# pikapuma/QuBLAS

Hardware: AMD Instinct MI355X
Metric: int-MAC/s (2*M*N*K/s) for Qgemul 4096^3 int<8,8>; % of MI355X int8 peak (higher is better)
Workload: dtype i8 limbs -> i32/i64; 1 GPU; 4096^3 Qgemul int<8,8> signed, linear class (MulArgs int17/frac16, AddArgs Qu<29,16>, C Qu<23,8>), 3x3 int8-limb MFMA; M_per_gpu=4096, N=4096, K=4096, class=linear

## Files before the change

### include/qgemul.h

```cpp
#ifndef QGEMUL_H_
#define QGEMUL_H_

#include <stddef.h>
#include <stdint.h>

#ifdef __cplusplus
extern "C" {
#endif

#define QGEMUL_ABI_VERSION 1u
#define QG_MAX_LEVELS 40

enum {
    QG_RND_POS_INF = 0,
    QG_RND_NEG_INF = 1,
    QG_RND_ZERO = 2,
    QG_RND_INF = 3,
    QG_RND_CONV = 4,
    QG_TRN_TCPL = 5,
    QG_TRN_SMGN = 6
};

enum {
    QG_SAT_TCPL = 0,
// ... 51 lines not shown
} qgemul_desc;

typedef struct qgemul_opts {
    int64_t lda, ldb, ldc;
    int32_t device;
    uint32_t flags;
} qgemul_opts;

enum {
    QG_OPT_FORCE_TREE = 1u,
    QG_OPT_CHECK_RANGE = 2u,
    QG_OPT_GENERIC_TREE = 4u,
    QG_OPT_RUNTIME_MODES = 8u,
    QG_OPT_FUSED_EPILOGUE = 16u,
    QG_OPT_UNFUSED_EPILOGUE = 32u,
    QG_OPT_GENERIC_LAYOUT = 64u,
    QG_OPT_SCHOOLBOOK_LIMBS = 2048u,
    QG_OPT_ARITHMETIC_CONV = 256u,
    QG_OPT_ALL_DEVICES = 512u,
    QG_OPT_BALANCED_LIMBS = 1024u,
    QG_OPT_LOCKSTEP_TILES = 128u,
    QG_OPT_APPROX_GENERAL = 4096u,
    QG_OPT_BATCHED_STACKED = 8192u,
    QG_OPT_BATCHED_TREE = 16384u
};

enum {
    QG_OK = 0,
    QG_EINVAL = -1,
    QG_EUNSUPPORTED = -2,
    QG_EHIP = -3,
    QG_ERCCL = -4,
    QG_ERANGE = -5,
    QG_ENOGPU = -6
};

enum {
    QG_CLASS_LINEAR = 1,
    QG_CLASS_TREE = 2
};

typedef struct qgemul_info {
    int32_t cls;
    int32_t supported;
    int32_t max_bits;
    int32_t in_bits[2];
    int32_t limbs[2];
// ... 255 lines not shown
```

### qublas_amd/build.py

```python
from __future__ import annotations

import os
import subprocess
import sys

HERE = os.path.dirname(os.path.abspath(__file__))
CSRC = os.path.join(HERE, "csrc")
SOURCES = ["qg_api.hip", "qg_run.hip", "qg_pack.hip", "qg_combine_bd.hip", "qg_eltwise.hip", "qg_approx.hip", "qg_eltwise_cplx.hip", "qg_tree.hip", "qg_tree_fast.hip", "qg_tree_fast_bd.hip", "qg_tree64.hip", "qg_tree_cplx.hip", "qg_tree_cplx_bd.hip", "qg_tree_rc.hip", "qg_gemv.hip", "qg_mfma.hip", "qg_mfma_ep_bd.hip", "qg_mfma_grp.hip", "qg_mfma_ep_grp.hip", "qg_mfma_pp.hip", "qg_mfma_ppl.hip", "qg_mfma_k6.hip", "qg_mfma_ring.hip", "qg_comm.hip", "qg_plan.cpp", "qg_geom.cpp"]
HEADERS = ["qg_ops.h", "qg_forms.h", "qg_plan.h", "qg_kernels.h", "qg_geom.h", "qg_tile_walk.h", "qg_grp.h", "qg_mfma_tile.h", "qg_member_forms.h", "qg_mfma_body.h", "qg_ring.h", "qg_step_all.h", "qg_tree_counter.h", "qg_tree_io.h", "qg_tree_bd.h", "qg_eltwise.h", "qg_eltwise_args.h", "qg_approx.h", "qg_approx_dev.h", "qg_cmul.h", "qg_fix.h", "qg_api_int.h", "qg_run_key.h", os.path.join("..", "..", "include", "qgemul.h")]
INCLUDED_UNITS = {"qg_tree_fast_bd.hip": ["qg_tree_fast.hip"], "qg_tree_cplx_bd.hip": ["qg_tree_cplx.hip"]}
FLAGS = ["--offload-arch=gfx950", "-O3", "-std=c++17", "-fPIC", "-Wall", "-Wno-unused-function", "-Wno-unused-value", "-Wno-unused-result", "-x", "hip"]
LIB = os.path.join(HERE, "libqugemm.so")
LIB_DIAG = os.path.join(HERE, "libqugemm_diag.so")


def _stale(obj: str, deps) -> bool:
    if not os.path.exists(obj):
        return True
    t = os.path.getmtime(obj)
    return any(os.path.getmtime(d) > t for d in deps if os.path.exists(d))


def build(force: bool = False, verbose: bool = False, diag: bool = False) -> str:
    hipcc = os.environ.get("HIPCC", "/opt/rocm/bin/hipcc")
    hdrs = [os.path.join(CSRC, h) for h in HEADERS]
    objdir = os.path.join(HERE, "build", "diag") if diag else os.path.join(HERE, "build")
    LIB = LIB_DIAG if diag else globals()["LIB"]
    os.makedirs(objdir, exist_ok=True)
    objs = []
    procs = []
    for s in SOURCES:
        src = os.path.join(CSRC, s)
# ... 21 lines not shown
```

### qublas_amd/capi.py

```python
from __future__ import annotations

import ctypes as C
import os
from typing import Optional

import numpy as np

from .desc import (QG_MAX_EW, Qcomplex, Qu, host_layout, qfmt, qgemul_approx, qgemul_approx_form, qgemul_approx_seg, qgemul_batched_ep, batched_ep, qgemul_grouped_ep, grouped_ep, qgemul_grouped_member, qgemul_cmul, qgemul_cmul_form, qgemul_desc, qgemul_ep_args, qgemul_epilogue,
                   qgemul_epilogue_cplx, qgemul_ew_stage, qgemul_info, qgemul_opts)

_HERE = os.path.dirname(os.path.abspath(__file__))
LIB_PATH = os.path.join(_HERE, "libqugemm_diag.so" if os.environ.get("QUBLAS_AMD_DIAG") == "1" else "libqugemm.so")

QG_OK, QG_EINVAL, QG_EUNSUPPORTED, QG_EHIP, QG_ERCCL, QG_ERANGE, QG_ENOGPU = 0, -1, -2, -3, -4, -5, -6
OPT_FORCE_TREE, OPT_CHECK_RANGE, OPT_GENERIC_TREE, OPT_RUNTIME_MODES, OPT_FUSED_EPILOGUE, OPT_UNFUSED_EPILOGUE = 1, 2, 4, 8, 16, 32
OPT_GENERIC_LAYOUT, OPT_LOCKSTEP_TILES, OPT_ARITHMETIC_CONV, OPT_ALL_DEVICES = 64, 128, 256, 512
OPT_SCHOOLBOOK_LIMBS = 2048
OPT_APPROX_GENERAL = 4096
OPT_BATCHED_TREE = 16384
OPT_BATCHED_STACKED = 8192
OPT_BALANCED_LIMBS = 1024
OPERAND_A, OPERAND_B, OPERAND_C = 0, 1, 2
BITS_ASCII, BITS_PACKED = 0, 1
KERNEL_NAMES = {0: "none", 1: "mfma_i8", 2: "mfma_i8_limb", 3: "tree_i32", 4: "tree_i64", 5: "tree_cplx", 6: "tree_cplx_i32", 7: "mfma_cplx", 8: "gemv_i32", 9: "gemv_i64", 10: "tree_i128", 11: "tree_rc_i32", 12: "mfma_rc"}
CMUL_NAMES = {0: "none", 1: "basic", 2: "tf", 3: "real_a", 4: "real_b"}

EXPORTS = [
    "qgemul_classify", "qgemul_strerror", "qgemul_abi_version", "qgemul_last_hip_error", "qgemul_run",
    "qgemul_ctx_create", "qgemul_ctx_destroy", "qgemul_ctx_sync", "qgemul_ctx_stream",
    "qgemul_plan_create", "qgemul_plan_destroy", "qgemul_plan_info",
    "qgemul_dev_alloc", "qgemul_dev_free", "qgemul_memcpy_h2d", "qgemul_memcpy_d2h",
    "qgemul_pack", "qgemul_pack_f64", "qgemul_unpack_c", "qgemul_execute", "qgemul_fill_packed", "qgemul_time_execute",
    "qgemul_classify_ep", "qgemul_plan_create_ep", "qgemul_packed_e_bytes", "qgemul_pack_e", "qgemul_execute_ep",
    "qgemul_time_execute_ep", "qgemul_run_ep", "qgemul_plan_fuses_epilogue", "qgemul_plan_packed_layout", "qgemul_classify_epc", "qgemul_plan_create_epc", "qgemul_run_epc",
    "qgemul_bitstream_bytes", "qgemul_export_bitstream", "qgemul_run_release", "qgemul_run_sharded", "qgemul_execute_host_c", "qgemul_plan_stores_host_c",
    "qgemul_comm_unique_id", "qgemul_comm_create", "qgemul_comm_destroy", "qgemul_comm_info", "qgemul_gather_packed_c", "qgemul_comm_fence",
    "qgemul_comm_sync", "qgemul_comm_barrier", "qgemul_comm_max_f64", "qgemul_last_rccl_error", "qgemul_ctx_device",
    "qgemul_classify_epx", "qgemul_plan_create_epx", "qgemul_run_epx", "qgemul_plan_approx_uniform", "qgemul_sizeof", "qgemul_approx_plan_form", "qgemul_apply_epilogue", "qgemul_time_apply_epilogue", "qgemul_packed_c_bytes", "qgemul_pack_c",
    "qgemul_classify_epcx", "qgemul_plan_create_epcx", "qgemul_run_epcx", "qgemul_cmul_plan_form",
    "qgemul_classify_batched", "qgemul_classify_batched_launches", "qgemul_plan_create_batched", "qgemul_plan_batched_launches", "qgemul_pack_batched",
    "qgemul_unpack_c_batched", "qgemul_execute_batched", "qgemul_time_execute_batched", "qgemul_time_execute_batched_launch", "qgemul_run_batched",
    "qgemul_classify_batched_epx", "qgemul_classify_batched_epx_launches", "qgemul_plan_create_batched_epx", "qgemul_pack_e_batched", "qgemul_execute_batched_ep",
# ... 779 lines not shown
```

### qublas_amd/csrc/qg_api.hip

```cpp
#include "qg_api_int.h"

static thread_local int g_last_hip = 0;
int qg_last_hip() { return g_last_hip; }
void qg_set_last_hip(int e) { g_last_hip = e; }

struct HostC { void* C; int64_t ld; };

template <class F>
static hipError_t comp_for_each_sub(const qgemul_plan* p, int operand, const QOperandGeom& g, F fn)
{
    const QComposite& q = p->comp;
    const int w = operand == QG_OPERAND_A ? 0 : 1;
    const QPackedGeom& base = w ? p->pb : p->pa;
    for (int c = 0; c < q.nc; ++c)
        for (int gi = 0; gi < (w ? q.gb : q.ga); ++gi) {
            int64_t off = 0;
            const QPackedGeom sp = qg_comp_sub_geom(q, base, w, p->desc.K, c, gi, &off);
            QOperandGeom sg = g;
            sg.k0 = (int64_t)c * q.kc;
            sg.K = qg_comp_chunk_len(q, p->desc.K, c);
            if (hipError_t e = fn(sg, sp, off); e != hipSuccess) return e;
        }
    return hipSuccess;
}
// ... 533 lines not shown
    QG_ON_DEVICE(p->ctx);
    QCGeom c = p->pc;
    c.ldc = ld ? ld : p->desc.M;
    QG_HIP(qg_launch_unpack_c(c, packed_dev, dst_dev, p->ctx->stream, (p->flags & QG_OPT_GENERIC_LAYOUT) ? 1 : 0));
    return QG_OK;
}

static int execute_kernel(qgemul_plan* p, void* packedC, const void* packedA, const void* packedB, const qgemul_ep_args* epa, const HostC* hostc = nullptr);

int qgemul_execute(qgemul_plan* p, void* packedC, const void* packedA, const void* packedB)
{
    if (!p || !packedC || !packedA || !packedB) return QG_EINVAL;
    if (p->batch) return QG_EINVAL;
    if (p->has_ep) return QG_EINVAL;
    if (p->desc.M == 0 || p->desc.N == 0) return QG_OK;
    QG_ON_DEVICE(p->ctx);
    return execute_kernel(p, packedC, packedA, packedB, nullptr);
}

bool stores_host_c(const qgemul_plan* p)
{
    if (p->has_ep || p->desc.is_complex || qg_wide_epilogue(p) || p->comp.on) return false;
    if (p->info.kernel != QG_KERNEL_MFMA_I8 && p->info.kernel != QG_KERNEL_MFMA_I8_LIMB) return false;
    if (p->variant != QG_MFMA_PP && p->variant != QG_MFMA_PPL && p->variant != QG_MFMA_K6) return false;
    if (p->variant == QG_MFMA_PPL && (p->pa.rows_p / p->cfg.TM) * (p->pb.rows_p / p->cfg.TN) < 256) return false;
    return (p->pc.cbytes == 4 || p->pc.cbytes == 8) && p->pc.cbytes == p->hc.size;
}

int qgemul_plan_stores_host_c(const qgemul_plan* p) { return p && stores_host_c(p) ? 1 : 0; }

int qgemul_execute_host_c(qgemul_plan* p, void* C_dev, int64_t ldc, const void* packedA, const void* packedB)
{
    if (!p || !C_dev || !packedA || !packedB || p->has_ep) return QG_EINVAL;
    if (p->batch) return QG_EINVAL;
    if (ldc && ldc < p->desc.M) return QG_EINVAL;
    if (p->desc.M == 0 || p->desc.N == 0) return QG_OK;
    QG_ON_DEVICE(p->ctx);
    if (stores_host_c(p)) {
        const HostC h{C_dev, ldc ? ldc : p->desc.M};
        return execute_kernel(p, C_dev, packedA, packedB, nullptr, &h);
    }
    if (!p->hostc_pc) QG_HIP(hipMalloc(&p->hostc_pc, (size_t)p->info.packed_bytes[2] ? (size_t)p->info.packed_bytes[2] : 16));
    const int st = execute_kernel(p, p->hostc_pc, packedA, packedB, nullptr);
    if (st != QG_OK) return st;
    QCGeom c = p->pc;
    c.ldc = ldc ? ldc : p->desc.M;
    QG_HIP(qg_launch_unpack_c(c, p->hostc_pc, C_dev, p->ctx->stream, (p->flags & QG_OPT_GENERIC_LAYOUT) ? 1 : 0));
// ... 1096 lines not shown
```

### qublas_amd/csrc/qg_geom.cpp

```cpp
#include "qg_geom.h"

#include <stdio.h>
#include <string.h>

#include <new>

int qg_pow2_bytes(int storage_bits)
{
    int b = (storage_bits + 7) / 8;
    int c = 1;
    while (c < b) c *= 2;
    return c;
}

QMfmaCfg qg_mfma_pick(int LA, int LB, int64_t M, int64_t N, uint32_t opt_flags)
{
    QMfmaCfg c = {QG_MFMA_NONE, 0, 0, 0};
    if (LA < 1 || LB < 1 || LA > 3 || LB > 3) return c;
    if (LA == 1 && LB == 1) {
        const int64_t big = ((M + 255) / 256) * ((N + 255) / 256);
        if (big >= 256) return (opt_flags & QG_OPT_LOCKSTEP_TILES) ? QMfmaCfg{QG_MFMA_256, 256, 256, 64} : QMfmaCfg{QG_MFMA_PP, 256, 256, 128};
        const int64_t mid = ((M + 127) / 128) * ((N + 127) / 128);
        static const bool no_small = QG_DIAG_ENV("QG_NO_SMALL_TILES");
        if (!no_small && mid <= 128 && ((M + 63) / 64) * ((N + 63) / 64) > mid) {
// ... 126 lines not shown
    const qgemul_desc* const d;
    const uint32_t flags;
    const EpView* const ev;
    const qgemul_epilogue* const ep;
    const int64_t batch;
    QPlanGeom* const out;
    QAnalysis* const an = &out->an;
    qgemul_info* const info = &out->info;
    QPackedGeom *const pa = &out->pa, *const pb = &out->pb;
    QCGeom* const pc = &out->pc;
    QHostElem* const hc = &out->hc;
    QComposite& comp = out->comp;
    const int parts = d->is_complex ? 2 : 1;
    const bool mixed = d->is_complex && (d->cmul == QG_CMUL_REAL_A || d->cmul == QG_CMUL_REAL_B);
    const int parts_a = d->is_complex && d->cmul != QG_CMUL_REAL_A ? 2 : 1, parts_b = d->is_complex && d->cmul != QG_CMUL_REAL_B ? 2 : 1;
    int LA = 0, LB = 0, kernel = QG_KERNEL_NONE;
    int64_t centreA = 0, centreB = 0;
    bool centred = false;
    QMfmaCfg cfg = {0, 0, 0, 0};
    bool bd = false;
    const bool want_stack = batch > 0 && (flags & QG_OPT_BATCHED_STACKED) && d->is_complex && !ev;
    bool stacked = false;
    bool k6 = false, ppl33 = false;


    int analysis_and_header()
    {
        out->bd = 0;
        out->bd_stack = QG_STACK_NONE;
        out->bd_tree = 0;
        memset(&comp, 0, sizeof comp);
        qg_analyze(d, an);
        memset(info, 0, sizeof *info);
        snprintf(info->reason, sizeof info->reason, "%s", an->reason);
        if (an->status != QG_OK) {
            info->supported = 0;
            return an->status;
        }
        out->ha = qg_host_elem(d->a, parts_a == 2);
        out->hb = qg_host_elem(d->b, parts_b == 2);
        *hc = qg_host_elem(d->c, d->is_complex);
        info->cls = an->cls;
        info->max_bits = an->max_bits;
        info->supported = 1;
        info->in_bits[0] = storage_bits(d->a, parts_a);
        info->in_bits[1] = storage_bits(d->b, parts_b);
// ... 82 lines not shown
            if (!comp.on) cfg = plain_cfg;
        }
    }

    void packed_c()
    {
        pc->M = d->M;
        pc->N = d->N;
        pc->parts = parts;
        pc->cbytes = qg_pow2_bytes(storage_bits(d->c, parts));
        if (an->band && pc->cbytes < (hc->sb[0] > hc->sb[1] ? hc->sb[0] : hc->sb[1])) pc->cbytes = hc->sb[0] > hc->sb[1] ? hc->sb[0] : hc->sb[1];
        pc->ldc = d->M;
        pc->elem_bytes = hc->size;
        for (int p = 0; p < 2; ++p) { pc->off[p] = hc->off[p]; pc->sb[p] = hc->sb[p]; }
    }

    void three_digit_choice()
    {
        static const bool no_kara3 = QG_DIAG_ENV("QG_NO_KARA3");
        const int cb = qg_pow2_bytes(storage_bits(d->c, parts));
        ppl33 = kernel == QG_KERNEL_MFMA_I8_LIMB && !comp.on && !d->is_complex && !ep && LA == 3 && LB == 3 && cfg.variant == QG_MFMA_PPL && (cb == 4 || cb == 8);
        k6 = ppl33 && !no_kara3 && !(flags & QG_OPT_SCHOOLBOOK_LIMBS) && !centred && !an->band && value_bits(d->a[0]) >= 13 && value_bits(d->a[0]) <= 18 &&
             value_bits(d->b[0]) >= 13 && value_bits(d->b[0]) <= 18 && d->K * (int64_t)(126 * 126) < (1ll << 31);
        if (k6) cfg = QMfmaCfg{QG_MFMA_K6, QG_K6_TM, QG_K6_TN, QG_K6_BK};
    }

    void limb_layout()
    {
        *pa = QPackedGeom{qg_round_up(d->M, cfg.TM), qg_round_up(d->K, cfg.BK), 1, LA, cfg.TM, cfg.BK};
        *pb = QPackedGeom{qg_round_up(d->N, cfg.TN), qg_round_up(d->K, cfg.BK), 1, LB, cfg.TN, cfg.BK};
        if (comp.on) {
            pa->K_p = pb->K_p = qg_round_up(comp.kc, cfg.BK);
            pa->limbs = comp.la[0];
            pb->limbs = comp.lb[0];
        }
        pc->Mp = pa->rows_p;
        pc->Np = pb->rows_p;
        pc->tm = cfg.TM;
        pc->tn = cfg.TN;
        if (k6) {
            pc->Mp = qg_round_up(d->M, 128);
            pc->tm = 128;
        }
        if (d->is_complex) {
            pc->Mp = d->M;
            pc->Np = d->N;
            pc->tm = pc->tn = 0;
// ... 66 lines not shown
    void digit6_layout()
    {
        QPackedGeom* g[2] = {pa, pb};
        for (int w = 0; w < 2; ++w) {
            const qfmt f = w ? d->b[0] : d->a[0];
            g[w]->digit6 = 1;
            g[w]->bias = f.S ? ((int64_t)1 << ((int)f.I + (int)f.F)) : 0;
            g[w]->rowsum_off = g[w]->trailer + QG_TRAILER_BYTES;
            info->packed_bytes[w] += g[w]->rows_p * 8;
        }
    }
    void digit_layouts()
    {
        if (!comp.on && !centred) {
            static const bool no_kara = QG_DIAG_ENV("QG_NO_KARA");
            if (!no_kara && !d->is_complex && LA == 2 && LB == 2 && (kernel == QG_KERNEL_MFMA_I8_LIMB) && (cfg.variant == QG_MFMA_LIMB_128 || cfg.variant == QG_MFMA_PPL) &&
                value_bits(d->a[0]) <= 12 && value_bits(d->b[0]) <= 12 && d->K * (int64_t)(126 * 126) < (1ll << 31)) {
                cfg.variant = QG_MFMA_LIMB_128;
                digit6_layout();
            }
        }
        if (k6) {
            digit6_layout();
            snprintf(info->reason, sizeof info->reason, "linear class: three base-64 digits per operand, six products (two-group kernel, 96x128 tiles)");
        } else if (ppl33) {
            snprintf(info->reason, sizeof info->reason, "linear class: balanced base-256 limbs, nine products (two-group kernel, 128x128 tiles)");
        }
    }

    int chain(QApproxTable* axt, QCmulStage* cmt)
    {
        if (an->band) return refuse(info, QG_EUNSUPPORTED, "element-wise chain after a plan whose C can leave its format (multi-word comparison artefact of the reference)");
        if ((d->is_complex != 0) != (ev->im != nullptr))
            return refuse(info, QG_EINVAL, d->is_complex ? "complex GEMM: the chain is a qgemul_epilogue_cplx" : "real GEMM: the chain is a qgemul_epilogue");
        QEpTable* const t[2] = {&out->ept, &out->ept_im};
        qfmt df[2] = {ep->d, ep->d};
        const bool lockstep = qg_view_has_cmul(ev);
        if (ev->cx && !lockstep)
            for (int k = 0; k < QG_MAX_EW; ++k)
                if (ev->cx[k]) return refuse(info, QG_EINVAL, "a CMUL record for a stage that is no CMUL stage");
        QEpTable both[2];
        for (int part = 0; part < parts; ++part) {
            const qgemul_epilogue* e = part ? ev->im : ep;
            int ep_bits = 0;
            char why[96];
            int st = QG_OK;
            if (lockstep) {
// ... 456 lines not shown
```

### qublas_amd/csrc/qg_geom.h

```cpp
#pragma once
#include <stdint.h>
#include <stdlib.h>

#include "qg_approx.h"
#include "qg_cmul.h"
#include "qg_grp.h"
#include "qg_plan.h"
#include "qg_run_key.h"

struct QOperandGeom {
    int64_t rows, K;
    int64_t rs, ks;
    int32_t elem_bytes;
    int32_t off[2], sb[2];
    int32_t parts;
    int32_t W[2], S[2];
    int32_t F[2], Q[2], O[2];
    int64_t k0;
};

struct QPackedGeom {
    int64_t rows_p, K_p;
    int32_t cbytes;
    int32_t limbs;
    int32_t tr, bk;
    int64_t trailer;
    int32_t digit6;
    int32_t limb0;
    int32_t offs, pad_;
    int64_t bias, rowsum_off;
};
enum { QG_TRAILER_BYTES = 256, QG_MASK_WORDS = 64 };

struct QCGeom {
    int64_t M, N, Mp, Np;
    int32_t tm, tn;
    int32_t cbytes;
    int32_t parts;
    int64_t ldc;
    int32_t elem_bytes, off[2], sb[2];
};

struct QMfmaCfg {
    int variant;
    int TM, TN, BK;
};
enum { QG_K6_VARIANT = 11, QG_K6_TM = 96, QG_K6_TN = 128, QG_K6_BK = 64 };
enum { QG_RING_VARIANT = 12, QG_RING_TM = 128, QG_RING_TN = 128, QG_RING_BK = 64 };
inline int qg_ring_digits(int n) { return (n + 7) / 8; }
inline int qg_ring_products(int LA, int LB, int L)
{
    int c = 0;
    for (int i = 0; i < LA; ++i)
        for (int j = 0; j < LB; ++j) c += i + j < L ? 1 : 0;
    return c;
}

enum QMfmaVariant {
    QG_MFMA_NONE = 0,
    QG_MFMA_128 = 1,
    QG_MFMA_256 = 2,
    QG_MFMA_LIMB_128 = 3,
    QG_MFMA_64 = 5,
    QG_MFMA_LIMB_64 = 6,
    QG_MFMA_64_BK128 = 7,
    QG_MFMA_128_BK128 = 8,
    QG_MFMA_PP = 9,
    QG_MFMA_PPL = 10,
    QG_MFMA_K6 = QG_K6_VARIANT,
    QG_MFMA_RING = QG_RING_VARIANT,
};

#ifdef QG_DIAG
#define QG_DIAG_ENV(name) (getenv(name) != nullptr)
#else
#define QG_DIAG_ENV(name) false
#endif

struct QComposite {
    int on;
    int ga, gb;
    int la[3], lb[3];
    int la0[3], lb0[3];
    int var[3][3];
    int nc;
    int64_t kc;
    int slab_bytes;
    int wide;
    int64_t chunk_bytes[2];
};
struct QPlanGeom {
    QAnalysis an;
    qgemul_info info;
// ... 88 lines not shown
```

### qublas_amd/csrc/qg_kernels.h

```cpp
#pragma once
#include <hip/hip_runtime.h>
#include <stddef.h>
#include <stdint.h>
#include <stdlib.h>

#include <atomic>

#include "qg_eltwise_args.h"
#include "qg_geom.h"
#include "qg_grp.h"
#include "qg_plan.h"
#include "qg_ring.h"

#if defined(__HIPCC__)
__device__ __forceinline__ unsigned qg_plane_mask(const uint32_t* m)
{
    if (!m) return 7u;
    unsigned v = m[threadIdx.x & 63];
#pragma unroll
    for (int o = 32; o; o >>= 1) v |= __shfl_xor(v, o);
    return (unsigned)__builtin_amdgcn_readfirstlane(v);
}
#endif

// ... 110 lines not shown
template <int I, class G>
QG_HD const G& qg_dependent(const G& g) { return g; }
struct QMfmaEpBdArgs : QMfmaArgs {
    QBdEp bd;
};
hipError_t qg_launch_mfma_ep_bd(int LA, int LB, const QMfmaEpBdArgs& a, int64_t batch, hipStream_t st);
hipError_t qg_launch_mfma_bd(int LA, int LB, const QMfmaArgs& a, int64_t batch, hipStream_t st);
struct QMfmaGrpArgs : QMfmaArgs {
    const QGrpTile* tiles;
};
hipError_t qg_launch_mfma_grp(int LA, int LB, const QMfmaGrpArgs& a, int64_t n_tiles, hipStream_t st);
struct QMfmaEpGrpArgs : QMfmaArgs {
    const QGrpTile* tiles;
    QGrpEp ge;
};
hipError_t qg_launch_mfma_ep_grp(int LA, int LB, const QMfmaEpGrpArgs& a, int64_t n_tiles, hipStream_t st);
hipError_t qg_launch_pack_member(const QOperandGeom& g, const QPackedGeom& p, const void* src, void* dst, int check_range, int* range_flag,
                                 hipStream_t st, int generic = 0);
hipError_t qg_launch_mfma_pp(const QMfmaArgs& a, hipStream_t st);
bool qg_mfma_ppl_applies(int LA, int LB, const QMfmaArgs& a);
hipError_t qg_launch_mfma_ppl(int limbs, const QMfmaArgs& a, hipStream_t st);
bool qg_mfma_k6_applies(const QMfmaArgs& a);
hipError_t qg_launch_mfma_k6(const QMfmaArgs& a, hipStream_t st);

inline hipError_t qg_lds_attr(const void* fn, int bytes, std::atomic<uint64_t>& done)
{
    int dev = 0;
    hipError_t e = hipGetDevice(&dev);
    if (e != hipSuccess) return e;
    if (dev >= 0 && dev < 64 && ((done.load(std::memory_order_acquire) >> dev) & 1)) return hipSuccess;
    e = hipFuncSetAttribute(fn, hipFuncAttributeMaxDynamicSharedMemorySize, bytes);
    if (e == hipSuccess && dev >= 0 && dev < 64) done.fetch_or(1ull << dev, std::memory_order_release);
    return e;
}

template <auto Kernel, class Args>
hipError_t qg_launch_lds(unsigned grid, unsigned block, int lds, hipStream_t st, const Args& a, int lds_max = 0)
{
    static std::atomic<uint64_t> attr_done{0};
    if (hipError_t e = qg_lds_attr((const void*)Kernel, lds_max ? lds_max : lds, attr_done); e != hipSuccess) return e;
    hipLaunchKernelGGL(Kernel, dim3(grid), dim3(block), lds, st, a);
    return hipGetLastError();
}

inline hipError_t qg_persistent_grid(int64_t tiles, unsigned* grid)
{
// ... 35 lines not shown
```

### qublas_amd/csrc/qg_mfma.hip

```cpp
#include <hip/hip_runtime.h>
#include <stdlib.h>

#include <utility>

#include "qg_eltwise.h"
#include "qg_kernels.h"
#include "qg_member_forms.h"
#include "qg_mfma_tile.h"
#include "qg_step_all.h"

namespace {

typedef int v16i __attribute__((ext_vector_type(16)));

template <int LA, int LB, int BK, int WGM, int WGN, int TI, int TJ, int NSTAGE, int ABL, bool EP, int SA = LA, int SB = LB, bool KARA = false, int KS = 1>
__global__ __launch_bounds__(64 * WGM * WGN * KS) void k_mfma(QMfmaArgs g)
{
    constexpr bool BD = false, GRP = false;
#include "qg_mfma_body.h"
}
template <int LA, int LB, int BK, int WGM, int WGN, int TI, int TJ, int NSTAGE, int SA = LA, int SB = LB>
__global__ __launch_bounds__(64 * WGM * WGN) void k_mfma_bd(QMfmaArgs g)
{
    constexpr int ABL = 0, KS = 1;
// ... 386 lines not shown
        if (blocks <= 0) return hipSuccess;
        if (blocks > 0x7fffffffll || a.Kp % F::BK || a.Mp != batch * a.bd_tm * F::TM || a.Np != batch * a.bd_tn * F::TN || a.has_ep || a.kara || a.c_host) return hipErrorInvalidValue;
        return qg_member_launch(form, a, [&](auto k) {
            using K = decltype(k);
            return qg_launch_lds<k_mfma_bd<QG_MEMBER_FORM_ARGS(K)>>((unsigned)blocks, K::THREADS, K::LDS, st, a);
        });
    });
}

#ifdef QG_DIAG
static int ablation()
{
    static int v = -1;
    if (v < 0) { const char* e = getenv("QG_ABLATE"); v = e ? atoi(e) : 0; }
    return v;
}
#else
static constexpr int ablation() { return 0; }
#endif

hipError_t qg_launch_mfma(int LA, int LB, const QMfmaArgs& a_in, hipStream_t st)
{
    if (a_in.variant == QG_MFMA_K6) return qg_launch_mfma_k6(a_in, st);
    if (a_in.variant == QG_MFMA_PPL && qg_mfma_ppl_applies(LA, LB, a_in)) return qg_launch_mfma_ppl(LA, a_in, st);
    QMfmaArgs a_v3;
    if (a_in.variant == QG_MFMA_PPL) { a_v3 = a_in; a_v3.variant = QG_MFMA_LIMB_128; }
    const QMfmaArgs& a = a_in.variant == QG_MFMA_PPL ? a_v3 : a_in;
#ifdef QG_DIAG
    if (const int abl = ablation(); abl > 0 && abl < 16) {
        if (LA == 3 && LB == 3 && a.variant == QG_MFMA_LIMB_128) {
            switch (abl) {
            case 1: return launch<3, 3, 64, 2, 4, 2, 1, 3, 1>(a, st);
            case 2: return launch<3, 3, 64, 2, 4, 2, 1, 3, 2>(a, st);
            case 3: return launch<3, 3, 64, 2, 4, 2, 1, 3, 3>(a, st);
            case 4: return launch<3, 3, 64, 2, 4, 2, 1, 3, 4>(a, st);
            case 6: return launch<3, 3, 64, 2, 4, 2, 1, 3, 6>(a, st);
            case 15: return launch<3, 3, 64, 2, 4, 2, 1, 3, 15>(a, st);
            default: return launch<3, 3, 64, 2, 4, 2, 1, 3, 5>(a, st);
            }
        }
        if (LA == 1 && LB == 1 && a.variant == QG_MFMA_256) {
            switch (abl) {
            case 1: return launch<1, 1, 64, 2, 4, 4, 2, 3, 1>(a, st);
            case 2: return launch<1, 1, 64, 2, 4, 4, 2, 3, 2>(a, st);
            case 3: return launch<1, 1, 64, 2, 4, 4, 2, 3, 3>(a, st);
            case 4: return launch<1, 1, 64, 2, 4, 4, 2, 3, 4>(a, st);
// ... 84 lines not shown
```

### qublas_amd/profmeta.py

```python
from __future__ import annotations

import hashlib
import json
import os
import subprocess

ROOT = os.path.dirname(os.path.dirname(os.path.abspath(__file__)))
CSRC = os.path.join(ROOT, "qublas_amd", "csrc")
KERNELS_JSON = os.path.join(ROOT, "profiles", "kernels.json")

COMMON = ["qg_ops.h", "qg_kernels.h"]
FAMILY_SOURCES = {
    "mfma_i8": ["qg_mfma.hip", "qg_mfma_pp.hip", "qg_mfma_ring.hip", "qg_ring.h", "qg_step_all.h"],
    "mfma_i8_limb": ["qg_mfma.hip", "qg_mfma_ppl.hip", "qg_mfma_k6.hip", "qg_mfma_ring.hip", "qg_ring.h", "qg_step_all.h"],
    "mfma_cplx": ["qg_mfma.hip", "qg_mfma_ppl.hip", "qg_step_all.h", "qg_pack.hip"],
    "tree_i32": ["qg_tree_fast.hip", "qg_tree_bd.h", "qg_tree_counter.h", "qg_tree_io.h", "qg_step_all.h", "qg_fix.h", "qg_forms.h"],
    "tree_i64": ["qg_tree64.hip", "qg_tree.hip", "qg_tree_counter.h", "qg_tree_io.h"],
    "tree_i128": ["qg_tree.hip", "qg_tree_io.h"],
    "tree_cplx": ["qg_tree.hip", "qg_tree_io.h"],
    "mfma_rc": ["qg_mfma.hip", "qg_mfma_ppl.hip", "qg_step_all.h", "qg_pack.hip"],
    "tree_rc_i32": ["qg_tree_rc.hip", "qg_tree_counter.h", "qg_tree_io.h", "qg_fix.h", "qg_forms.h"],
    "tree_cplx_i32": ["qg_tree_cplx.hip", "qg_tree_bd.h", "qg_tree_counter.h", "qg_tree_io.h", "qg_fix.h", "qg_forms.h"],
    "gemv_i32": ["qg_gemv.hip", "qg_tree_io.h", "qg_fix.h", "qg_forms.h"],
    "gemv_i64": ["qg_gemv.hip", "qg_tree_io.h", "qg_fix.h", "qg_forms.h"],
}


def source_hashes(engine_kernel: str) -> dict:
    out = {}
    for f in FAMILY_SOURCES.get(engine_kernel, []) + COMMON:
        p = os.path.join(CSRC, f)
        out[f] = hashlib.sha256(open(p, "rb").read()).hexdigest()[:16] if os.path.exists(p) else None
    return out


def git_head() -> str:
    try:
# ... 27 lines not shown
```

Baseline: 459900 billion int-op/s (2*M*N*K/s).

## Add K7 kernel: seven products on five accumulator sets with 128x128 tiles

```diff
diff --git a/include/qgemul.h b/include/qgemul.h
--- a/include/qgemul.h
+++ b/include/qgemul.h
@@ -97,7 +97,9 @@
     QG_OPT_LOCKSTEP_TILES = 128u,
     QG_OPT_APPROX_GENERAL = 4096u,
     QG_OPT_BATCHED_STACKED = 8192u,
-    QG_OPT_BATCHED_TREE = 16384u
+    QG_OPT_BATCHED_TREE = 16384u,
+    QG_OPT_K6_TILES = 32768u,
+    QG_OPT_K7_TILES = 65536u
 };
 
 enum {
diff --git a/qublas_amd/build.py b/qublas_amd/build.py
--- a/qublas_amd/build.py
+++ b/qublas_amd/build.py
@@ -6,8 +6,8 @@
 
 HERE = os.path.dirname(os.path.abspath(__file__))
 CSRC = os.path.join(HERE, "csrc")
-SOURCES = ["qg_api.hip", "qg_run.hip", "qg_pack.hip", "qg_combine_bd.hip", "qg_eltwise.hip", "qg_approx.hip", "qg_eltwise_cplx.hip", "qg_tree.hip", "qg_tree_fast.hip", "qg_tree_fast_bd.hip", "qg_tree64.hip", "qg_tree_cplx.hip", "qg_tree_cplx_bd.hip", "qg_tree_rc.hip", "qg_gemv.hip", "qg_mfma.hip", "qg_mfma_ep_bd.hip", "qg_mfma_grp.hip", "qg_mfma_ep_grp.hip", "qg_mfma_pp.hip", "qg_mfma_ppl.hip", "qg_mfma_k6.hip", "qg_mfma_ring.hip", "qg_comm.hip", "qg_plan.cpp", "qg_geom.cpp"]
-HEADERS = ["qg_ops.h", "qg_forms.h", "qg_plan.h", "qg_kernels.h", "qg_geom.h", "qg_tile_walk.h", "qg_grp.h", "qg_mfma_tile.h", "qg_member_forms.h", "qg_mfma_body.h", "qg_ring.h", "qg_step_all.h", "qg_tree_counter.h", "qg_tree_io.h", "qg_tree_bd.h", "qg_eltwise.h", "qg_eltwise_args.h", "qg_approx.h", "qg_approx_dev.h", "qg_cmul.h", "qg_fix.h", "qg_api_int.h", "qg_run_key.h", os.path.join("..", "..", "include", "qgemul.h")]
+SOURCES = ["qg_api.hip", "qg_run.hip", "qg_pack.hip", "qg_combine_bd.hip", "qg_eltwise.hip", "qg_approx.hip", "qg_eltwise_cplx.hip", "qg_tree.hip", "qg_tree_fast.hip", "qg_tree_fast_bd.hip", "qg_tree64.hip", "qg_tree_cplx.hip", "qg_tree_cplx_bd.hip", "qg_tree_rc.hip", "qg_gemv.hip", "qg_mfma.hip", "qg_mfma_ep_bd.hip", "qg_mfma_grp.hip", "qg_mfma_ep_grp.hip", "qg_mfma_pp.hip", "qg_mfma_ppl.hip", "qg_mfma_k6.hip", "qg_mfma_k7.hip", "qg_mfma_ring.hip", "qg_comm.hip", "qg_plan.cpp", "qg_geom.cpp"]
+HEADERS = ["qg_ops.h", "qg_forms.h", "qg_plan.h", "qg_kernels.h", "qg_geom.h", "qg_tile_walk.h", "qg_k7_pieces.h", "qg_grp.h", "qg_mfma_tile.h", "qg_member_forms.h", "qg_mfma_body.h", "qg_ring.h", "qg_step_all.h", "qg_tree_counter.h", "qg_tree_io.h", "qg_tree_bd.h", "qg_eltwise.h", "qg_eltwise_args.h", "qg_approx.h", "qg_approx_dev.h", "qg_cmul.h", "qg_fix.h", "qg_api_int.h", "qg_run_key.h", os.path.join("..", "..", "include", "qgemul.h")]
 INCLUDED_UNITS = {"qg_tree_fast_bd.hip": ["qg_tree_fast.hip"], "qg_tree_cplx_bd.hip": ["qg_tree_cplx.hip"]}
 FLAGS = ["--offload-arch=gfx950", "-O3", "-std=c++17", "-fPIC", "-Wall", "-Wno-unused-function", "-Wno-unused-value", "-Wno-unused-result", "-x", "hip"]
 LIB = os.path.join(HERE, "libqugemm.so")
diff --git a/qublas_amd/capi.py b/qublas_amd/capi.py
--- a/qublas_amd/capi.py
+++ b/qublas_amd/capi.py
@@ -18,6 +18,8 @@
 OPT_SCHOOLBOOK_LIMBS = 2048
 OPT_APPROX_GENERAL = 4096
 OPT_BATCHED_TREE = 16384
+OPT_K6_TILES = 32768
+OPT_K7_TILES = 65536
 OPT_BATCHED_STACKED = 8192
 OPT_BALANCED_LIMBS = 1024
 OPERAND_A, OPERAND_B, OPERAND_C = 0, 1, 2
diff --git a/qublas_amd/csrc/qg_api.hip b/qublas_amd/csrc/qg_api.hip
--- a/qublas_amd/csrc/qg_api.hip
+++ b/qublas_amd/csrc/qg_api.hip
@@ -579,7 +579,7 @@
 {
     if (p->has_ep || p->desc.is_complex || qg_wide_epilogue(p) || p->comp.on) return false;
     if (p->info.kernel != QG_KERNEL_MFMA_I8 && p->info.kernel != QG_KERNEL_MFMA_I8_LIMB) return false;
-    if (p->variant != QG_MFMA_PP && p->variant != QG_MFMA_PPL && p->variant != QG_MFMA_K6) return false;
+    if (p->variant != QG_MFMA_PP && p->variant != QG_MFMA_PPL && p->variant != QG_MFMA_K6 && p->variant != QG_MFMA_K7) return false;
     if (p->variant == QG_MFMA_PPL && (p->pa.rows_p / p->cfg.TM) * (p->pb.rows_p / p->cfg.TN) < 256) return false;
     return (p->pc.cbytes == 4 || p->pc.cbytes == 8) && p->pc.cbytes == p->hc.size;
 }
diff --git a/qublas_amd/csrc/qg_geom.cpp b/qublas_amd/csrc/qg_geom.cpp
--- a/qublas_amd/csrc/qg_geom.cpp
+++ b/qublas_amd/csrc/qg_geom.cpp
@@ -172,6 +172,7 @@
     const bool want_stack = batch > 0 && (flags & QG_OPT_BATCHED_STACKED) && d->is_complex && !ev;
     bool stacked = false;
     bool k6 = false, ppl33 = false;
+    bool k7 = false;
 
 
     int analysis_and_header()
@@ -300,7 +301,9 @@
         ppl33 = kernel == QG_KERNEL_MFMA_I8_LIMB && !comp.on && !d->is_complex && !ep && LA == 3 && LB == 3 && cfg.variant == QG_MFMA_PPL && (cb == 4 || cb == 8);
         k6 = ppl33 && !no_kara3 && !(flags & QG_OPT_SCHOOLBOOK_LIMBS) && !centred && !an->band && value_bits(d->a[0]) >= 13 && value_bits(d->a[0]) <= 18 &&
              value_bits(d->b[0]) >= 13 && value_bits(d->b[0]) <= 18 && d->K * (int64_t)(126 * 126) < (1ll << 31);
-        if (k6) cfg = QMfmaCfg{QG_MFMA_K6, QG_K6_TM, QG_K6_TN, QG_K6_BK};
+        static const bool no_k7 = QG_DIAG_ENV("QG_NO_K7");
+        k7 = k6 && batch == 0 && !no_k7 && !(flags & QG_OPT_K6_TILES) && ((flags & QG_OPT_K7_TILES) || qg_k7_faster(d->M, d->N));
+        if (k6) cfg = QMfmaCfg{k7 ? QG_MFMA_K7 : QG_MFMA_K6, QG_K6_TM, QG_K6_TN, QG_K6_BK};
     }
 
     void limb_layout()
@@ -413,7 +416,8 @@
         }
         if (k6) {
             digit6_layout();
-            snprintf(info->reason, sizeof info->reason, "linear class: three base-64 digits per operand, six products (two-group kernel, 96x128 tiles)");
+            snprintf(info->reason, sizeof info->reason, k7 ? "linear class: 3 base-64 digits, seven products on five sets, 128x128 tiles (or six products)"
+                                                           : "linear class: three base-64 digits per operand, six products (two-group kernel, 96x128 tiles)");
         } else if (ppl33) {
             snprintf(info->reason, sizeof info->reason, "linear class: balanced base-256 limbs, nine products (two-group kernel, 128x128 tiles)");
         }
diff --git a/qublas_amd/csrc/qg_geom.h b/qublas_amd/csrc/qg_geom.h
--- a/qublas_amd/csrc/qg_geom.h
+++ b/qublas_amd/csrc/qg_geom.h
@@ -46,6 +46,14 @@
     int TM, TN, BK;
 };
 enum { QG_K6_VARIANT = 11, QG_K6_TM = 96, QG_K6_TN = 128, QG_K6_BK = 64 };
+enum { QG_K7_VARIANT = 13, QG_K7_TM = 128, QG_K7_TN = 128 };
+enum { QG_K7_ROUND = 256, QG_K7_TILE_RATIO_NUM = 151, QG_K7_TILE_RATIO_DEN = 100 };
+inline bool qg_k7_faster(int64_t M, int64_t N)
+{
+    const int64_t tn = (N + 127) / 128;
+    const int64_t r6 = (((M + 95) / 96) * tn + QG_K7_ROUND - 1) / QG_K7_ROUND, r7 = (((M + 127) / 128) * tn + QG_K7_ROUND - 1) / QG_K7_ROUND;
+    return r7 * QG_K7_TILE_RATIO_NUM < r6 * QG_K7_TILE_RATIO_DEN;
+}
 enum { QG_RING_VARIANT = 12, QG_RING_TM = 128, QG_RING_TN = 128, QG_RING_BK = 64 };
 inline int qg_ring_digits(int n) { return (n + 7) / 8; }
 inline int qg_ring_products(int LA, int LB, int L)
@@ -69,6 +77,7 @@
     QG_MFMA_PPL = 10,
     QG_MFMA_K6 = QG_K6_VARIANT,
     QG_MFMA_RING = QG_RING_VARIANT,
+    QG_MFMA_K7 = QG_K7_VARIANT,
 };
 
 #ifdef QG_DIAG
diff --git a/qublas_amd/csrc/qg_k7_pieces.h b/qublas_amd/csrc/qg_k7_pieces.h
--- /dev/null
+++ b/qublas_amd/csrc/qg_k7_pieces.h
@@ -0,0 +1,26 @@
+#pragma once
+#include <stdint.h>
+
+#ifndef QG_HD
+#if defined(__HIPCC__)
+#define QG_HD __host__ __device__ __forceinline__
+#else
+#define QG_HD inline
+#endif
+#endif
+
+enum {
+    QG_K7_PACK_TM = 96,
+    QG_K7_PIECE_ROWS = 16,
+    QG_K7_PIECE_BYTES = 16 * 64,
+    QG_K7_PLANE_A = QG_K7_PACK_TM * 64,
+    QG_K7_KTILE_A = 3 * QG_K7_PLANE_A
+};
+
+QG_HD int64_t qg_k7_piece_base(int64_t R0, int g, int64_t Mp, int64_t nk)
+{
+    int64_t r = R0 + (int64_t)QG_K7_PIECE_ROWS * g;
+    if (r > Mp - QG_K7_PIECE_ROWS) r = Mp - QG_K7_PIECE_ROWS;
+    const int64_t tile = r / QG_K7_PACK_TM, piece = (r % QG_K7_PACK_TM) / QG_K7_PIECE_ROWS;
+    return tile * nk * QG_K7_KTILE_A + piece * QG_K7_PIECE_BYTES;
+}
diff --git a/qublas_amd/csrc/qg_kernels.h b/qublas_amd/csrc/qg_kernels.h
--- a/qublas_amd/csrc/qg_kernels.h
+++ b/qublas_amd/csrc/qg_kernels.h
@@ -156,6 +156,8 @@
 hipError_t qg_launch_mfma_ppl(int limbs, const QMfmaArgs& a, hipStream_t st);
 bool qg_mfma_k6_applies(const QMfmaArgs& a);
 hipError_t qg_launch_mfma_k6(const QMfmaArgs& a, hipStream_t st);
+bool qg_mfma_k7_applies(const QMfmaArgs& a);
+hipError_t qg_launch_mfma_k7(const QMfmaArgs& a, hipStream_t st);
 
 inline hipError_t qg_lds_attr(const void* fn, int bytes, std::atomic<uint64_t>& done)
 {
diff --git a/qublas_amd/csrc/qg_mfma.hip b/qublas_amd/csrc/qg_mfma.hip
--- a/qublas_amd/csrc/qg_mfma.hip
+++ b/qublas_amd/csrc/qg_mfma.hip
@@ -432,6 +432,7 @@
 hipError_t qg_launch_mfma(int LA, int LB, const QMfmaArgs& a_in, hipStream_t st)
 {
     if (a_in.variant == QG_MFMA_K6) return qg_launch_mfma_k6(a_in, st);
+    if (a_in.variant == QG_MFMA_K7) return qg_launch_mfma_k7(a_in, st);
     if (a_in.variant == QG_MFMA_PPL && qg_mfma_ppl_applies(LA, LB, a_in)) return qg_launch_mfma_ppl(LA, a_in, st);
     QMfmaArgs a_v3;
     if (a_in.variant == QG_MFMA_PPL) { a_v3 = a_in; a_v3.variant = QG_MFMA_LIMB_128; }
diff --git a/qublas_amd/csrc/qg_mfma_k7.hip b/qublas_amd/csrc/qg_mfma_k7.hip
--- /dev/null
+++ b/qublas_amd/csrc/qg_mfma_k7.hip
@@ -0,0 +1,284 @@
+#include <hip/hip_runtime.h>
+
+#include <type_traits>
+
+#include "qg_k7_pieces.h"
+#include "qg_kernels.h"
+#include "qg_mfma_tile.h"
+#include "qg_step_all.h"
+
+namespace {
+
+constexpr int TM = 128, TN = 128, BK = 64;
+constexpr int PLANE = TM * BK;
+constexpr int BUF = 6 * PLANE;
+constexpr int NBUF = 3;
+constexpr uint32_t H = 0x80808080u;
+
+__device__ __forceinline__ uint64_t k7_recombine(uint32_t c0, uint32_t c1, uint32_t c2, uint32_t c3, uint32_t c4, uint64_t base)
+{
+    uint32_t m6 = 1u << 6, m12 = 1u << 12, m18 = 1u << 18, m24 = 1u << 24;
+    asm("" : "+s"(m6), "+s"(m12), "+s"(m18), "+s"(m24));
+    uint64_t x = base + c0;
+    x = (uint64_t)c1 * m6 + x;
+    x = (uint64_t)c2 * m12 + x;
+    x = (uint64_t)c3 * m18 + x;
+    return (uint64_t)c4 * m24 + x;
+}
+
+template <int NV, int... P>
+__device__ __forceinline__ void k7_pace(std::integer_sequence<int, P...>)
+{
+    (((void)P, __builtin_amdgcn_sched_group_barrier(0x008, 1, 0), __builtin_amdgcn_sched_group_barrier(0x002, NV, 0)), ...);
+}
+
+template <bool FAST, int CB>
+__global__ __launch_bounds__(512) void k_mfma_k7(QMfmaArgs g)
+{
+    extern __shared__ __attribute__((aligned(16))) char smem[];
+    const int lane = threadIdx.x & 63;
+    const int wave = __builtin_amdgcn_readfirstlane(threadIdx.x >> 6);
+    const int wm = wave >> 2, wn = wave & 3;
+
+    const int tiles_m = (int)(g.Mc / TM), tiles_n = (int)(g.Np / TN);
+    const int nwg = tiles_m * tiles_n;
+    const QTileList my = qg_tile_list(nwg, blockIdx, gridDim);
+    const int n_my = my.count;
+    if (n_my == 0) return;
+
+    const int nk = (int)(g.Kp / BK);
+    const int64_t panel_b = (int64_t)nk * 3 * PLANE;
+    uint32_t lane16 = (uint32_t)(lane * 16);
+    char* const lds_w = smem + wave * 1024;
+    struct Cursor { const int8_t* a; const int8_t* b; int kt, ti; };
+    auto cursor_at_tile = [&](int ti) {
+        int tm, tn;
+        qg_tile_of<8>(my.first + ti * my.step, tiles_m, tiles_n, tm, tn);
+        return Cursor{g.A + qg_k7_piece_base((int64_t)tm * TM, wave, g.Mp, nk), g.B + tn * panel_b + wave * 1024, 0, ti};
+    };
+    auto advance = [&](Cursor c) {
+        if (c.kt + 1 < nk) return Cursor{c.a + QG_K7_KTILE_A, c.b + 3 * PLANE, c.kt + 1, c.ti};
+        if (c.ti + 1 < n_my) return cursor_at_tile(c.ti + 1);
+        return c;
+    };
+    auto issue_a = [&](int buf_off, int l, const Cursor& c) {
+        __builtin_amdgcn_global_load_lds(QG_GLOBAL_PTR(c.a + l * QG_K7_PLANE_A + lane16), QG_LDS_PTR(lds_w + buf_off + l * PLANE), 16, 0, 0);
+    };
+    auto issue_b = [&](int buf_off, int l, const Cursor& c) {
+        __builtin_amdgcn_global_load_lds(QG_GLOBAL_PTR(c.b + l * PLANE + lane16), QG_LDS_PTR(lds_w + buf_off + (3 + l) * PLANE), 16, 0, 0);
+    };
+
+    enum { C0, C1, C3, C4, ZM, NACC };
+    v4i acc[NACC][4][2];
+    const int fr = lane & 15, fq = lane >> 4;
+    const int chunk = (fq ^ qg_swz<64>(fr)) * 16;
+    const int a_lane = (wm * 64 + fr) * BK + chunk;
+    const int b_lane = 3 * PLANE + (wn * 32 + fr) * BK + chunk;
+    v4i fa[3][4], fb[3][2];
+    typedef const __attribute__((address_space(3))) v4i* LdsFrag;
+    const uint32_t lds0 = (uint32_t)(uintptr_t)QG_LDS_PTR(smem);
+    uint32_t rd_a = lds0 + a_lane, rd_b = lds0 + b_lane;
+    auto read_ab = [&](int l) {
+#pragma unroll
+        for (int i = 0; i < 4; ++i) fa[l][i] = *(LdsFrag)(uintptr_t)(rd_a + l * PLANE + i * (16 * BK));
+#pragma unroll
+        for (int j = 0; j < 2; ++j) fb[l][j] = *(LdsFrag)(uintptr_t)(rd_b + l * PLANE + j * (16 * BK));
+    };
+    auto mfma = [&](int s, int la, int i, int lb, int j) {
+        acc[s][i][j] = __builtin_amdgcn_mfma_i32_16x16x64_i8(fa[la][i], fb[lb][j], acc[s][i][j], 0, 0, 0);
+    };
+    auto product = [&](int s, int la, int lb) {
+#pragma unroll
+        for (int i = 0; i < 4; ++i)
+#pragma unroll
+            for (int j = 0; j < 2; ++j) mfma(s, la, i, lb, j);
+    };
+    auto issue_tile = [&](int buf_off, const Cursor& c) {
+        issue_b(buf_off, 0, c);
+        issue_a(buf_off, 0, c);
+        issue_b(buf_off, 1, c);
+        issue_a(buf_off, 1, c);
+        issue_b(buf_off, 2, c);
+        issue_a(buf_off, 2, c);
+    };
+#define QG_LOAD_DONE(N)                                             \
+    do {                                                            \
+        asm volatile("s_waitcnt vmcnt(" #N ")" ::: "memory");       \
+        asm volatile("s_waitcnt lgkmcnt(0)" ::: "memory");          \
+        __builtin_amdgcn_sched_barrier(0);                          \
+        __builtin_amdgcn_s_barrier();                               \
+        __builtin_amdgcn_sched_barrier(0);                          \
+    } while (0)
+#define QG_MFMA_DONE()                                              \
+    do {                                                            \
+        __builtin_amdgcn_s_setprio(0);                              \
+        __builtin_amdgcn_sched_barrier(0);                          \
+        __builtin_amdgcn_s_barrier();                               \
+        __builtin_amdgcn_sched_barrier(0);                          \
+    } while (0)
+
+    Cursor nxt = cursor_at_tile(0);
+    issue_tile(0, nxt);
+    nxt = advance(nxt);
+    issue_tile(BUF, nxt);
+    nxt = advance(nxt);
+    asm volatile("s_waitcnt vmcnt(6)" ::: "memory");
+    __builtin_amdgcn_s_barrier();
+    asm volatile("" ::: "memory");
+
+    int cur = 0, fill = 2 * BUF;
+    for (int ti = 0; ti < n_my; ++ti) {
+#pragma unroll
+        for (int s = 0; s < NACC; ++s)
+#pragma unroll
+            for (int i = 0; i < 4; ++i)
+#pragma unroll
+                for (int j = 0; j < 2; ++j)
+#pragma unroll
+                    for (int e = 0; e < 4; ++e) acc[s][i][j][e] = 0;
+        if (wm == 1) __builtin_amdgcn_s_barrier();
+        __builtin_amdgcn_sched_barrier(0);
+
+        for (int kt = 0; kt < nk; ++kt) {
+            asm volatile("" : "+v"(lane16));
+            read_ab(0);
+            read_ab(1);
+            read_ab(2);
+            issue_tile(fill, nxt);
+            QG_LOAD_DONE(6);
+            __builtin_amdgcn_s_setprio(1);
+#pragma unroll
+            for (int i = 0; i < 4; ++i) {
+                mfma(C0, 0, i, 0, 0);
+                mfma(C0, 0, i, 0, 1);
+                mfma(C1, 0, i, 1, 0);
+                mfma(C1, 0, i, 1, 1);
+            }
+#pragma unroll
+            for (int i = 0; i < 4; ++i) fa[0][i] = ((fa[0][i] | (int)H) - fa[1][i] + fa[2][i]) ^ (int)H;
+            product(C1, 1, 0);
+#pragma unroll
+            for (int j = 0; j < 2; ++j) fb[0][j] = ((fb[0][j] | (int)H) - fb[1][j] + fb[2][j]) ^ (int)H;
+            product(C3, 1, 2);
+            product(C3, 2, 1);
+            product(C4, 2, 2);
+            product(ZM, 0, 0);
+            const int t = cur, step = cur + BUF == NBUF * BUF ? -(NBUF - 1) * BUF : BUF;
+            cur += step;
+            fill = t;
+            rd_a += step;
+            rd_b += step;
+            asm volatile("" : "+v"(rd_a), "+v"(rd_b));
+            k7_pace<2>(std::make_integer_sequence<int, 48>{});
+            __builtin_amdgcn_sched_group_barrier(0x002, 2, 0);
+            __builtin_amdgcn_sched_group_barrier(0x008, 8, 0);
+            QG_MFMA_DONE();
+            nxt = advance(nxt);
+        }
+        if (wm == 0) __builtin_amdgcn_s_barrier();
+        __builtin_amdgcn_sched_barrier(0);
+
+        int efr = fr, efq = fq;
+        asm volatile("" : "+v"(efr), "+v"(efq));
+        int tile_m, tile_n;
+        qg_tile_of<8>(my.first + ti * my.step, tiles_m, tiles_n, tile_m, tile_n);
+        const QStep st = g.to_c;
+        char* C = (char*)g.C;
+        const int64_t tile_base = ((int64_t)tile_m * tiles_n + tile_n) * TM * TN;
+        [[maybe_unused]] const int sh = st.d;
+        uint64_t colt[2], rowt[4][4];
+#pragma unroll
+        for (int j = 0; j < 2; ++j) colt[j] = (uint64_t)g.rsB[(int64_t)tile_n * TN + wn * 32 + j * 16 + efr];
+#pragma unroll
+        for (int i = 0; i < 4; ++i)
+#pragma unroll
+            for (int e = 0; e < 4; ++e) {
+                const int64_t r = (int64_t)tile_m * TM + wm * 64 + i * 16 + 4 * efq + e;
+                rowt[i][e] = (uint64_t)g.rsA[r < g.Mp ? r : g.Mp - 1];
+            }
+#pragma unroll
+        for (int j = 0; j < 2; ++j) colt[j] = (uint64_t)g.corr - (uint64_t)g.biasA * colt[j];
+#pragma unroll
+        for (int i = 0; i < 4; ++i)
+#pragma unroll
+            for (int e = 0; e < 4; ++e) rowt[i][e] = (uint64_t)g.biasB * rowt[i][e];
+#pragma unroll
+        for (int i = 0; i < 4; ++i) {
+            int64_t s[8];
+#pragma unroll
+            for (int j = 0; j < 2; ++j)
+#pragma unroll
+                for (int e = 0; e < 4; ++e) {
+                    const uint32_t c0 = (uint32_t)acc[C0][i][j][e], c1 = (uint32_t)acc[C1][i][j][e], c3 = (uint32_t)acc[C3][i][j][e],
+                                   c4 = (uint32_t)acc[C4][i][j][e];
+                    const uint32_t c2 = (uint32_t)acc[ZM][i][j][e] - c0 + c1 + c3 - c4;
+                    s[j * 4 + e] = (int64_t)k7_recombine(c0, c1, c2, c3, c4, colt[j] - rowt[i][e]);
+                }
+            if constexpr (FAST) {
+#pragma unroll
+                for (int o = 0; o < 8; ++o) {
+                    const int64_t x = s[o] >> sh, y = x < st.lo ? st.lo : x;
+                    s[o] = y > st.hi ? st.hi : y;
+                }
+            } else {
+                qg_step_all<int64_t, 8>(s, st);
+            }
+            const int row0 = wm * 64 + i * 16 + 4 * efq;
+            const int64_t gr = (int64_t)tile_m * TM + row0;
+#pragma unroll
+            for (int j = 0; j < 2; ++j) {
+                const int col = wn * 32 + j * 16 + efr;
+                const int64_t* q = s + j * 4;
+                if (g.c_host) {
+                    const int64_t gc = (int64_t)tile_n * TN + col;
+                    if (gc < g.c_N) {
+                        using E = std::conditional_t<CB == 4, int32_t, int64_t>;
+                        E* dst = (E*)C + gc * g.c_ld + gr;
+                        if (gr + 3 < g.c_M && g.c_vec) {
+                            if constexpr (CB == 4) *(int4*)dst = make_int4((int)q[0], (int)q[1], (int)q[2], (int)q[3]);
+                            else { *(longlong2*)dst = make_longlong2(q[0], q[1]); *(longlong2*)(dst + 2) = make_longlong2(q[2], q[3]); }
+                        } else {
+#pragma unroll
+                            for (int e = 0; e < 4; ++e)
+                                if (gr + e < g.c_M) dst[e] = (E)q[e];
+                        }
+                    }
+                    continue;
+                }
+                if (gr >= g.Mp) continue;
+                qg_store_run4<CB>(C, tile_base + (int64_t)col * TM + row0, q);
+            }
+        }
+    }
+    asm volatile("s_waitcnt vmcnt(0)" ::: "memory");
+#undef QG_LOAD_DONE
+#undef QG_MFMA_DONE
+}
+
+template <bool FAST, int CB>
+hipError_t launch_k7(const QMfmaArgs& a, unsigned grid, hipStream_t st)
+{
+    return qg_launch_lds<k_mfma_k7<FAST, CB>>(grid, 512, NBUF * BUF, st, a);
+}
+
+}
+
+bool qg_mfma_k7_applies(const QMfmaArgs& a)
+{
+    if (a.has_ep || !a.kara || a.variant != QG_MFMA_K7 || !a.rsA || !a.rsB) return false;
+    if (a.cbytes != 4 && a.cbytes != 8) return false;
+    return a.Kp > 0 && a.Kp % BK == 0 && a.Mp >= QG_K7_PACK_TM && a.Mp % QG_K7_PACK_TM == 0 && a.Np % TN == 0 && a.Mc > 0 && a.Mc % TM == 0 && a.Mc <= a.Mp + 127;
+}
+
+hipError_t qg_launch_mfma_k7(const QMfmaArgs& a, hipStream_t st)
+{
+    if (!qg_mfma_k7_applies(a)) return hipErrorInvalidValue;
+    const int64_t blocks = (a.Mc / TM) * (a.Np / TN);
+    if (blocks <= 0) return hipSuccess;
+    if (blocks > 0x7fffffffll) return hipErrorInvalidValue;
+    unsigned grid = 0;
+    if (hipError_t e = qg_persistent_grid(blocks, &grid); e != hipSuccess) return e;
+    const bool fast = qg_step_is_shift_clamp(a.to_c);
+    if (a.cbytes == 4) return fast ? launch_k7<true, 4>(a, grid, st) : launch_k7<false, 4>(a, grid, st);
+    return fast ? launch_k7<true, 8>(a, grid, st) : launch_k7<false, 8>(a, grid, st);
+}
diff --git a/qublas_amd/profmeta.py b/qublas_amd/profmeta.py
--- a/qublas_amd/profmeta.py
+++ b/qublas_amd/profmeta.py
@@ -12,7 +12,7 @@
 COMMON = ["qg_ops.h", "qg_kernels.h"]
 FAMILY_SOURCES = {
     "mfma_i8": ["qg_mfma.hip", "qg_mfma_pp.hip", "qg_mfma_ring.hip", "qg_ring.h", "qg_step_all.h"],
-    "mfma_i8_limb": ["qg_mfma.hip", "qg_mfma_ppl.hip", "qg_mfma_k6.hip", "qg_mfma_ring.hip", "qg_ring.h", "qg_step_all.h"],
+    "mfma_i8_limb": ["qg_mfma.hip", "qg_mfma_ppl.hip", "qg_mfma_k6.hip", "qg_mfma_k7.hip", "qg_mfma_ring.hip", "qg_ring.h", "qg_step_all.h"],
     "mfma_cplx": ["qg_mfma.hip", "qg_mfma_ppl.hip", "qg_step_all.h", "qg_pack.hip"],
     "tree_i32": ["qg_tree_fast.hip", "qg_tree_bd.h", "qg_tree_counter.h", "qg_tree_io.h", "qg_step_all.h", "qg_fix.h", "qg_forms.h"],
     "tree_i64": ["qg_tree64.hip", "qg_tree.hip", "qg_tree_counter.h", "qg_tree_io.h"],
```

Result: no change. 459900 billion int-op/s (2*M*N*K/s) (median of 2 runs) (-0.0%).
